# raulmur/ORB_SLAM

Hardware: NVIDIA H100
Metric: Mkeypoints/s extract+match (higher is better)
Workload: dtype u8

## Files before the change

orb_slam_b200/csrc/extract_kernels.cu:

```cuda
#include <cuda_fp16.h>

#include "orbfe_internal.h"

namespace orbfe {

__global__ void cell_select_harris_kernel(const PlanDev *__restrict__ plan, WorkDev wk, int f0);
__global__ void level_select_harris_kernel(const PlanDev *__restrict__ plan, WorkDev wk, int f0);

__device__ __forceinline__ int find_level_by(const PlanDev *plan, int idx, int which) {
    int l = 0;
    const int n = plan->nlevels;
    for (int k = 1; k < n; k++) {
        const LevelDev &L = plan->lv[k];
        const int base = which == 0 ? L.ftile_base : which == 1 ? L.btile_base : which == 2 ? L.cell_base : L.kp_base;
        if (idx >= base) l = k;
    }
    return l;
}

__device__ __forceinline__ void pdl_prologue() {
    asm volatile("griddepcontrol.launch_dependents;" ::: "memory");
    asm volatile("griddepcontrol.wait;" ::: "memory");
}

// ... 107 lines not shown
#undef RZ_PIX_SEL
#undef RZ_MIX
        if (y < dh) *reinterpret_cast<uint32_t *>(dst + (size_t)y * D.pitch) = out;
    }
}

void launch_resize_level(const PlanDev *d_plan, const PlanDev &hp, int level, int f0, int nf, cudaStream_t s) {
    const LevelDev &D = hp.lv[level];
    dim3 block(64, 4);
    dim3 grid((D.w + 255) / 256, (D.h + 4 * RZ_ROWS - 1) / (4 * RZ_ROWS), nf);
    launch_k(resize_level_kernel, grid, block, 0, s, hp.pdl != 0, d_plan, level, f0);
}

#define F2_W ORBFE_FT_W
#define F2_H ORBFE_FT_H
#define F2_PW 144
#define F2_PWORDS 35
#define F2_PH (F2_H + 8)
#define F2_MS 128
#ifndef ORBFE_FAST_ARC_DEFAULT
#define ORBFE_FAST_ARC_DEFAULT 12
#endif
#define F2_MH (F2_H + 2)
static_assert(F2_MH == 64, "the m tile is 8 warps x 8 rows; row 64 does not exist (ti.hmask has 64 bits)");

__device__ __forceinline__ uint32_t max16_u16x2(const uint32_t *w) {
    const uint32_t a0 = __vimax3_u16x2(w[0], w[1], w[2]), a1 = __vimax3_u16x2(w[3], w[4], w[5]);
    const uint32_t a2 = __vimax3_u16x2(w[6], w[7], w[8]), a3 = __vimax3_u16x2(w[9], w[10], w[11]);
    const uint32_t a4 = __vimax3_u16x2(w[12], w[13], w[14]);
    return __vmaxu2(__vimax3_u16x2(a0, a1, a2), __vimax3_u16x2(a3, a4, w[15]));
}
__device__ __forceinline__ uint32_t min16_u16x2(const uint32_t *w) {
    const uint32_t a0 = __vimin3_u16x2(w[0], w[1], w[2]), a1 = __vimin3_u16x2(w[3], w[4], w[5]);
    const uint32_t a2 = __vimin3_u16x2(w[6], w[7], w[8]), a3 = __vimin3_u16x2(w[9], w[10], w[11]);
    const uint32_t a4 = __vimin3_u16x2(w[12], w[13], w[14]);
    return __vminu2(__vimin3_u16x2(a0, a1, a2), __vimin3_u16x2(a3, a4, w[15]));
}

__device__ __forceinline__ uint32_t fast_m_u16x2(const uint32_t (&r)[16], uint32_t c) {
    uint32_t tmin[16], tmax[16], w[16];
#pragma unroll
    for (int k = 0; k < 16; k++) {
        tmin[k] = __vimin3_u16x2(r[k], r[(k + 1) & 15], r[(k + 2) & 15]);
        tmax[k] = __vimax3_u16x2(r[k], r[(k + 1) & 15], r[(k + 2) & 15]);
    }
#pragma unroll
    for (int k = 0; k < 16; k++) w[k] = __vimin3_u16x2(tmin[k], tmin[(k + 3) & 15], tmin[(k + 6) & 15]);
// ... 62 lines not shown
template <int ARC>
__device__ __forceinline__ uint32_t fast_m_arc(const uint32_t (&r)[16], uint32_t c) {
    if (ARC < 0) return fast_m_u16x2(r, c);
    return fast_m2_u16x2<(ARC < 0 ? 0 : ARC)>(r, c);
}

__device__ __forceinline__ void fast_load_row(const uint8_t *row , uint32_t (&P)[8]) {
    const uint32_t w0 = *reinterpret_cast<const uint32_t *>(row);
    const uint32_t w1 = *reinterpret_cast<const uint32_t *>(row + 4);
    const uint32_t w2 = *reinterpret_cast<const uint32_t *>(row + 8);
    const uint32_t E0 = __byte_perm(w0, 0, 0x4240), O0 = __byte_perm(w0, 0, 0x4341);
    const uint32_t E1 = __byte_perm(w1, 0, 0x4240), O1 = __byte_perm(w1, 0, 0x4341);
    const uint32_t E2 = __byte_perm(w2, 0, 0x4240), O2 = __byte_perm(w2, 0, 0x4341);
    P[0] = O0;
    P[1] = __byte_perm(E0, E1, 0x5412);
    P[2] = __byte_perm(O0, O1, 0x5412);
    P[3] = E1;
    P[4] = O1;
    P[5] = __byte_perm(E1, E2, 0x5412);
    P[6] = __byte_perm(O1, O2, 0x5412);
    P[7] = E2;
}

__device__ __forceinline__ int m_at(const uint32_t *mt, int r, int c ) {
    const int g = c >> 2, k = c & 3;
    const uint32_t wv = mt[(r * 32 + g) * 2 + (k & 1)];
    return (k & 2) ? (int)(wv >> 16) : (int)(wv & 0xFFFF);
}

#define F2_MAXC ((F2_W / 2) * (F2_H / 2) + 4 * (F2_W + F2_H))
#define F2_MAXCELLS 64

__device__ __forceinline__ uint32_t float_order_key(float v) {
    const uint32_t b = __float_as_uint(v);
    return (b & 0x80000000u) ? ~b : (b | 0x80000000u);
}
__device__ __forceinline__ float float_from_order_key(uint32_t k) {
    return __uint_as_float((k & 0x80000000u) ? (k & 0x7FFFFFFFu) : ~k);
}

__device__ __forceinline__ float harris_response(const uint8_t *__restrict__ img, int pitch, int x, int y, float scale4) {
    int a = 0, b = 0, c = 0;
    for (int i = -3; i <= 3; i++) {
        const uint8_t *r0 = img + (size_t)(y + i - 1) * pitch + x, *r1 = r0 + pitch, *r2 = r1 + pitch;
        for (int j = -3; j <= 3; j++) {
            const int Ix = ((int)__ldg(r1 + j + 1) - (int)__ldg(r1 + j - 1)) * 2 + ((int)__ldg(r0 + j + 1) - (int)__ldg(r0 + j - 1)) +
                           ((int)__ldg(r2 + j + 1) - (int)__ldg(r2 + j - 1));
            const int Iy = ((int)__ldg(r2 + j) - (int)__ldg(r0 + j)) * 2 + ((int)__ldg(r2 + j - 1) - (int)__ldg(r0 + j - 1)) +
                           ((int)__ldg(r2 + j + 1) - (int)__ldg(r0 + j + 1));
            a += Ix * Ix;
            b += Iy * Iy;
// ... 2 lines not shown
    }
    const float fa = (float)a, fb = (float)b, fc = (float)c;
    const float s = __fadd_rn(fa, fb);
    const float t = __fsub_rn(__fsub_rn(__fmul_rn(fa, fb), __fmul_rn(fc, fc)), __fmul_rn(__fmul_rn(0.04f, s), s));
    return __fmul_rn(t, scale4);
}

__device__ __forceinline__ void fast_push(uint32_t *q, int *q_n, int xl, int yl, int m) {
    const int n = atomicAdd(q_n, 1);
    q[n] = (uint32_t)xl | ((uint32_t)yl << 7) | ((uint32_t)m << 13);
}

__device__ __forceinline__ void cell_window(const LevelDev &L, int xmax, int ymax, int x, int y, int &ci, int &cj, int &xa,
                                            int &xb, int &ya, int &yb) {
    cj = min((int)__umulhi((uint32_t)(x - ORBFE_EDGE), L.cw_rcp), L.cols - 1);
    ci = min((int)__umulhi((uint32_t)(y - ORBFE_EDGE), L.ch_rcp), L.rows - 1);
    xa = ORBFE_EDGE + cj * L.cw;
    ya = ORBFE_EDGE + ci * L.ch;
    xb = (cj == L.cols - 1) ? xmax - 1 : xa + L.cw - 1;
    yb = (ci == L.rows - 1) ? ymax - 1 : ya + L.ch - 1;
}

template <int PSTRIDE, int ARC>
__device__ __forceinline__ void fast_tile_compute(const PlanDev *__restrict__ plan, const WorkDev &wk, int tile, int level, int f, int x0, int y0, const uint8_t *pix, uint32_t *mt,
                                                  uint32_t *s_cand, int &s_n, int *s_cnt_lo, int *s_cnt_hi,
                                                  long long *s_kbase, int *s_klim) {
    const int tlo = plan->t_lo;
    const int g = threadIdx.x & 31, seg = threadIdx.x >> 5;
    const int gx = x0 - 4 + 4 * g;
    {
        const int xmax = plan->lv[level].w - ORBFE_EDGE, ymax = plan->lv[level].h - ORBFE_EDGE;
        uint32_t keepA = 0, keepB = 0;
        if (gx >= ORBFE_EDGE && gx < xmax) keepA |= 0x00003C00u;
        if (gx + 2 >= ORBFE_EDGE && gx + 2 < xmax) keepA |= 0x3C000000u;
        if (gx + 1 >= ORBFE_EDGE && gx + 1 < xmax) keepB |= 0x00003C00u;
        if (gx + 3 >= ORBFE_EDGE && gx + 3 < xmax) keepB |= 0x3C000000u;
        const uint32_t ntlo2 = (uint32_t)tlo * 0x00010001u | 0x80008000u;
        uint32_t yin_bits = 0;
#pragma unroll
        for (int i = 0; i < 8; i++) {
            const int y = y0 - 1 + seg * 8 + i;
            if (y >= ORBFE_EDGE && y < ymax) yin_bits |= 1u << i;
        }
        const uint8_t *base = &pix[(seg * 8) * PSTRIDE + 4 * g];
        uint32_t P[7][8];
#pragma unroll
        for (int r = 0; r < 6; r++) fast_load_row(base + r * PSTRIDE, P[r]);
#pragma unroll
        for (int i = 0; i < 8; i++) {
            fast_load_row(base + (6 + i) * PSTRIDE, P[(6 + i) % 7]);
#define FROW(dy) P[(i + (dy) + 3) % 7]
            uint32_t mA, mB;
            {
                const uint32_t r[16] = {FROW(3)[3], FROW(3)[4], FROW(2)[5], FROW(1)[6], FROW(0)[6], FROW(-1)[6], FROW(-2)[5], FROW(-3)[4],
                                        FROW(-3)[3], FROW(-3)[2], FROW(-2)[1], FROW(-1)[0], FROW(0)[0], FROW(1)[0], FROW(2)[1], FROW(3)[2]};
                mA = fast_m_arc<ARC>(r, FROW(0)[3]);
            }
            {
                const uint32_t r[16] = {FROW(3)[4], FROW(3)[5], FROW(2)[6], FROW(1)[7], FROW(0)[7], FROW(-1)[7], FROW(-2)[6], FROW(-3)[5],
                                        FROW(-3)[4], FROW(-3)[3], FROW(-2)[2], FROW(-1)[1], FROW(0)[1], FROW(1)[1], FROW(2)[2], FROW(3)[3]};
                mB = fast_m_arc<ARC>(r, FROW(0)[4]);
            }
#undef FROW
            const int mr = seg * 8 + i;
            const bool yin = (yin_bits >> i) & 1u;
            uint2 o;
            o.x = hfma2_relu(mA, yin ? keepA : 0u, ntlo2);
            o.y = hfma2_relu(mB, yin ? keepB : 0u, ntlo2);
            *reinterpret_cast<uint2 *>(&mt[(mr * 32 + g) * 2]) = o;
        }
    }
    __syncthreads();
    const FTileInfo &ti = wk.ftile_info[tile];
    const LevelDev &L = plan->lv[ti.level];
    const int xmax = L.w - ORBFE_EDGE, ymax = L.h - ORBFE_EDGE;
    const int thi = plan->t_hi;
    uint32_t fbits = 0;
    const int r0 = seg * 8;
    uint32_t vb;
    {
        const uint32_t nib = (ti.vmask[g >> 3] >> (4 * (g & 7))) & 15u;
        vb = nib | (__shfl_down_sync(0xffffffffu, nib, 1) & 1u) << 4;
    }
    if (g >= 1 && g <= 30) {
        const uint32_t ONE2 = 0x3C003C00u, NEG2 = 0xBC00BC00u;
        const uint32_t kLA = ((vb & 1u) ? 0u : 0x00003C00u) | ((vb & 4u) ? 0u : 0x3C000000u);
        const uint32_t kM = ((vb & 2u) ? 0u : 0x00003C00u) | ((vb & 8u) ? 0u : 0x3C000000u);
        const uint32_t kRB = ((vb & 4u) ? 0u : 0x00003C00u) | ((vb & 16u) ? 0u : 0x3C000000u);
        const uint32_t nkM = kM | 0x80008000u;
        const uint32_t hm = (uint32_t)(ti.hmask >> r0);
        uint32_t A[3], B[3], lrA[3], lrB[3], fullA[3], fullB[3];
#pragma unroll
        for (int j = 0; j < 10; j++) {
            const int rr = j == 0 ? max(r0 - 1, 0) : j == 9 ? min(r0 + 8, F2_MH - 1) : r0 - 1 + j;
            const uint32_t *rowp = &mt[(rr * 32 + g) * 2];
            const uint2 own = *reinterpret_cast<const uint2 *>(rowp);
            const uint32_t pB = rowp[-1], nA = rowp[2];
            const int sl = j % 3;
            A[sl] = own.x;
            B[sl] = own.y;
            const uint32_t leftA = hmul2(__byte_perm(pB, own.y, 0x5432), kLA);
            const uint32_t rightB = hmul2(__byte_perm(own.x, nA, 0x5432), kRB);
            lrA[sl] = hmax2_keep(leftA, own.y, kM, nkM);
            fullA[sl] = hmax2_keep(lrA[sl], own.x, ONE2, NEG2);
            lrB[sl] = hmax2_keep(rightB, own.x, kM, nkM);
            fullB[sl] = hmax2_keep(lrB[sl], own.y, ONE2, NEG2);
            if (j >= 2) {
                const int c = (j - 1) % 3, u = (j - 2) % 3, d = j % 3;
                const uint32_t kUp = ((hm >> (j - 2)) & 1u) ? 0u : ONE2, kDn = ((hm >> (j - 1)) & 1u) ? 0u : ONE2;
                const uint32_t eA = hfma2(A[c], NEG2, hmax2_keep(hmax2_keep(lrA[c], fullA[d], kDn, kDn | 0x80008000u), fullA[u], kUp, kUp | 0x80008000u));
                const uint32_t eB = hfma2(B[c], NEG2, hmax2_keep(hmax2_keep(lrB[c], fullB[d], kDn, kDn | 0x80008000u), fullB[u], kUp, kUp | 0x80008000u));
                fbits |= (__byte_perm(eA, eB, 0x7351) & 0x80808080u) >> (7 - (j - 2));
            }
        }
        if (seg == 0) fbits &= 0xFEFEFEFEu;
        if (seg == 7) fbits &= 0x7F7F7F7Fu;
    }
    {
        {
            const int mine = __popc(fbits);
            int incl = mine;
#pragma unroll
            for (int o = 1; o < 32; o <<= 1) {
                const int v = __shfl_up_sync(0xffffffffu, incl, o);
                if (g >= o) incl += v;
            }
            int wbase = 0;
            const int total = __shfl_sync(0xffffffffu, incl, 31);
            if (g == 31 && total) wbase = atomicAdd(&s_n, total);
            wbase = __shfl_sync(0xffffffffu, wbase, 31);
            int n = wbase + incl - mine;
            while (fbits) {
                const int b = __ffs(fbits) - 1;
                fbits &= fbits - 1;
                const int cr = r0 + (b & 7), k = b >> 3;
                s_cand[n++] = (uint32_t)(gx + k - x0) | ((uint32_t)(cr - 1) << 7) | ((uint32_t)(m_at(mt, cr, 4 * g + k) + tlo) << 13);
            }
        }
    }
    __syncthreads();
    const int ncand = s_n;
    const int ncell_loc = ti.ncj * ti.nci;
    for (int i = threadIdx.x; i < ncand; i += blockDim.x) {
        const uint32_t q = s_cand[i];
        const int x = x0 + (int)(q & 127), y = y0 + (int)((q >> 7) & 63), m = (int)((q >> 13) & 255);
        int ci, cj, xa, xb, ya, yb;
        cell_window(L, xmax, ymax, x, y, ci, cj, xa, xb, ya, yb);
        const int lc = (ci - ti.ci0) * ti.ncj + (cj - ti.cj0);
        const int slot = atomicAdd(&s_cnt_lo[lc], 1);
        if (m > thi) atomicAdd(&s_cnt_hi[lc], 1);
        if (slot >= 2048) atomicExch(wk.err_flag, 3);
        s_cand[i] = q | ((uint32_t)slot << 21);
    }
    __syncthreads();
    if ((int)threadIdx.x < ncell_loc) {
        const int lc = threadIdx.x;
        const int gcell = L.cell_base + (ti.ci0 + lc / ti.ncj) * L.cols + (ti.cj0 + lc % ti.ncj);
        const size_t fc = (size_t)f * plan->ncells_total + gcell;
        const int cap = wk.cell_cand_cap[gcell];
// ... 7 lines not shown
        s_klim[lc] = cap - base;
    }
    __syncthreads();
    for (int i = threadIdx.x; i < ncand; i += blockDim.x) {
        const uint32_t q = s_cand[i];
        const int x = x0 + (int)(q & 127), y = y0 + (int)((q >> 7) & 63), m = (int)((q >> 13) & 255), slot = (int)(q >> 21);
        int ci, cj, xa, xb, ya, yb;
        cell_window(L, xmax, ymax, x, y, ci, cj, xa, xb, ya, yb);
        const int lc = (ci - ti.ci0) * ti.ncj + (cj - ti.cj0);
        const uint32_t raster = (uint32_t)((y - ya) * L.cw + (x - xa));
        if (slot < s_klim[lc]) {
            const size_t kidx = (size_t)(s_kbase[lc] + slot);
            if (wk.cand_keys64) {
                const float resp = harris_response(L.pyr + (size_t)f * L.plane, L.pitch, x, y, plan->harris_scale4);
                wk.cand_keys64[kidx] = ((unsigned long long)float_order_key(resp) << 32) |
                                       ((unsigned long long)(0xFFFFFFu - raster) << 8) | (unsigned long long)(m - 1);
            } else {
                wk.cand_keys[kidx] = ((uint32_t)(m - 1) << 24) | (0xFFFFFFu - raster);
            }
        }
    }
}

__global__ void __launch_bounds__(256, 2) fast_nms_kernel(const PlanDev *__restrict__ plan, WorkDev wk, int f0) {
    __shared__ __align__(16) uint8_t sbuf[(F2_MAXC * 4 > F2_PH * F2_PW) ? F2_MAXC * 4 : F2_PH * F2_PW];
    __shared__ __align__(16) uint32_t mt[F2_MH * 32 * 2];
    __shared__ int s_n, s_cnt_lo[F2_MAXCELLS], s_cnt_hi[F2_MAXCELLS], s_klim[F2_MAXCELLS];
    __shared__ long long s_kbase[F2_MAXCELLS];
    uint8_t *pix = sbuf;
    uint32_t *s_cand = reinterpret_cast<uint32_t *>(sbuf);

    const int f = blockIdx.y + f0;
    const FTileInfo ti = wk.ftile_info[blockIdx.x];
    const LevelDev &L = plan->lv[ti.level];
    const int x0 = ORBFE_EDGE + ti.tx * F2_W, y0 = ORBFE_EDGE + ti.ty * F2_H;
    const int h = L.h, pitch = L.pitch;
    const uint8_t *__restrict__ img = L.pyr + (size_t)f * L.plane;

    if (threadIdx.x < F2_MAXCELLS) { s_cnt_lo[threadIdx.x] = 0; s_cnt_hi[threadIdx.x] = 0; }
    if (threadIdx.x == 0) s_n = 0;
    {
        const int max_word = pitch / 4 - 1;
        const int wx0 = (x0 - 8) >> 2;
        for (int i = threadIdx.x; i < F2_PH * F2_PWORDS; i += blockDim.x) {
            const int r = i / F2_PWORDS, c = i - r * F2_PWORDS;
            const int gy = min(y0 - 4 + r, h - 1);
            const int gw = min(wx0 + c, max_word);
            *reinterpret_cast<uint32_t *>(&pix[r * F2_PW + c * 4]) =
                __ldg(reinterpret_cast<const uint32_t *>(img + (size_t)gy * pitch) + gw);
        }
    }
    __syncthreads();
    fast_tile_compute<F2_PW, ORBFE_FAST_ARC_DEFAULT>(plan, wk, blockIdx.x, ti.level, f, x0, y0, pix, mt, s_cand, s_n, s_cnt_lo, s_cnt_hi, s_kbase, s_klim);
}

__device__ __forceinline__ uint32_t smem_u32(const void *p) { return (uint32_t)__cvta_generic_to_shared(p); }

__device__ __forceinline__ void mbar_init(uint64_t *bar, int count) {
    asm volatile("mbarrier.init.shared::cta.b64 [%0], %1;" ::"r"(smem_u32(bar)), "r"(count));
}
__device__ __forceinline__ void mbar_expect_tx(uint64_t *bar, uint32_t bytes) {
    asm volatile("mbarrier.arrive.expect_tx.shared::cta.b64 _, [%0], %1;" ::"r"(smem_u32(bar)), "r"(bytes) : "memory");
}
__device__ __forceinline__ void mbar_wait(uint64_t *bar, uint32_t parity) {
    asm volatile(
        "{\n"
        ".reg .pred p;\n"
        "WAIT_%=:\n"
        "mbarrier.try_wait.parity.shared::cta.b64 p, [%0], %1;\n"
        "@p bra DONE_%=;\n"
        "bra WAIT_%=;\n"
        "DONE_%=:\n"
        "}\n" ::"r"(smem_u32(bar)), "r"(parity) : "memory");
}
__device__ __forceinline__ void tma_load_3d(void *smem_dst, const void *tmap, uint64_t *bar, int c0, int c1, int c2) {
    asm volatile(
        "cp.async.bulk.tensor.3d.shared::cluster.global.mbarrier::complete_tx::bytes [%0], [%1, {%3, %4, %5}], [%2];"
        ::"r"(smem_u32(smem_dst)), "l"(tmap), "r"(smem_u32(bar)), "r"(c0), "r"(c1), "r"(c2) : "memory");
}

#define F2_TW 160
#define F2_PIXBYTES (F2_PH * F2_TW)
#define F2_PIXSLOT ((F2_PIXBYTES + 127) / 128 * 128)
#define F2_TMA_SMEM (2 * F2_PIXSLOT + F2_MH * 32 * 2 * 4 + 128)
static_assert(F2_MAXC * 4 <= F2_PIXSLOT, "the candidate queue lives in the pixel slot that was just consumed");

template <int ARC, int MINB>
__global__ void __launch_bounds__(256, MINB) fast_nms_tma_kernel(const PlanDev *__restrict__ plan, WorkDev wk, int f0, int nwork) {
    extern __shared__ __align__(128) uint8_t dsm[];
    uint8_t *pixbuf0 = dsm, *pixbuf1 = dsm + F2_PIXSLOT;
    uint32_t *mt = reinterpret_cast<uint32_t *>(dsm + 2 * F2_PIXSLOT);
    __shared__ __align__(8) uint64_t bar[2];
    __shared__ int s_n, s_cnt_lo[F2_MAXCELLS], s_cnt_hi[F2_MAXCELLS], s_klim[F2_MAXCELLS];
    __shared__ long long s_kbase[F2_MAXCELLS];

    const int ntiles = plan->nftiles_total;
    if (threadIdx.x == 0) {
        mbar_init(&bar[0], 1);
        mbar_init(&bar[1], 1);
        asm volatile("fence.mbarrier_init.release.cluster;" ::: "memory");
    }
    __syncthreads();
    pdl_prologue();
    int wi = blockIdx.x;
    if (wi < nwork && threadIdx.x == 0) {
        const FTileInfo t0 = wk.ftile_info[wi % ntiles];
        mbar_expect_tx(&bar[0], F2_PIXBYTES);
        tma_load_3d(pixbuf0, &wk.tmaps[t0.level], &bar[0], (ORBFE_EDGE + t0.tx * F2_W - 8) & ~15, ORBFE_EDGE + t0.ty * F2_H - 4, f0 + wi / ntiles);
    }
    for (int it = 0; wi < nwork; it++, wi += gridDim.x) {
        const int cur = it & 1;
        const int nxt = wi + gridDim.x;
        const FTileInfo ti = wk.ftile_info[wi % ntiles];
        const int f = f0 + wi / ntiles;
        const int x0 = ORBFE_EDGE + ti.tx * F2_W, y0 = ORBFE_EDGE + ti.ty * F2_H;
        if (threadIdx.x < F2_MAXCELLS) { s_cnt_lo[threadIdx.x] = 0; s_cnt_hi[threadIdx.x] = 0; }
        if (threadIdx.x == 0) s_n = 0;
        mbar_wait(&bar[cur], (it >> 1) & 1);
        __syncthreads();
        if (nxt < nwork && threadIdx.x == 0) {
            const FTileInfo tn = wk.ftile_info[nxt % ntiles];
            mbar_expect_tx(&bar[cur ^ 1], F2_PIXBYTES);
            tma_load_3d(cur ? pixbuf0 : pixbuf1, &wk.tmaps[tn.level], &bar[cur ^ 1], (ORBFE_EDGE + tn.tx * F2_W - 8) & ~15,
                        ORBFE_EDGE + tn.ty * F2_H - 4, f0 + nxt / ntiles);
        }
        uint8_t *slot_cur = cur ? pixbuf1 : pixbuf0;
        fast_tile_compute<F2_TW, ARC>(plan, wk, wi % ntiles, ti.level, f, x0, y0, slot_cur + ((x0 - 8) & 15), mt, reinterpret_cast<uint32_t *>(slot_cur),
                                 s_n, s_cnt_lo, s_cnt_hi, s_kbase, s_klim);
    }
}

#define FAST_ARC_VARIANTS(X) X(-1, 4) X(0, 4) X(4, 4) X(8, 4) X(12, 4) X(16, 4) X(12, 3) X(16, 3)
typedef void (*FastTmaKernel)(const PlanDev *, WorkDev, int, int);
static FastTmaKernel fast_tma_variant(int arc, int minb) {
#define X(a, b) if (arc == (a) && minb == (b)) return fast_nms_tma_kernel<(a), (b)>;
    FAST_ARC_VARIANTS(X)
#undef X
    return nullptr;
}
int fast_arc_supported(int arc, int ctas_per_sm) { return fast_tma_variant(arc, ctas_per_sm <= 3 ? 3 : 4) != nullptr; }

int fast_tma_setup() {
#define X(a, b) { cudaError_t e = cudaFuncSetAttribute(fast_nms_tma_kernel<(a), (b)>, cudaFuncAttributeMaxDynamicSharedMemorySize, F2_TMA_SMEM); if (e != cudaSuccess) return (int)e; }
    FAST_ARC_VARIANTS(X)
#undef X
    return 0;
}

void launch_fast_nms(const PlanDev *d_plan, const PlanDev &hp, WorkDev w, int f0, int nf, cudaStream_t s) {
    if (hp.nftiles_total == 0) return;
    if (w.tmaps) {
        const int nwork = hp.nftiles_total * nf;
        const int grid = min(nwork, w.fast_grid);
        launch_k(fast_tma_variant(w.fast_arc, w.fast_ctas <= 3 ? 3 : 4), dim3(grid), dim3(256), F2_TMA_SMEM, s, hp.pdl != 0, d_plan, w, f0, nwork);
        return;
    }
    dim3 grid(hp.nftiles_total, nf);
    fast_nms_kernel<<<grid, 256, 0, s>>>(d_plan, w, f0);
}

__device__ __forceinline__ int warp_sum(int v) {
#pragma unroll
    for (int o = 16; o > 0; o >>= 1) v += __shfl_xor_sync(0xffffffffu, v, o);
    return v;
}

__global__ void __launch_bounds__(32) cell_quota_kernel(const PlanDev *__restrict__ plan, WorkDev wk, int f0) {
    pdl_prologue();
    __shared__ uint32_t no_more[128];
    const int l = blockIdx.x, f = blockIdx.y + f0;
    const LevelDev &L = plan->lv[l];
    const int lane = threadIdx.x;
    const int nCells = L.ncells, nfc = L.nfc;
    const size_t fb = (size_t)f * plan->ncells_total + L.cell_base;
    const int t1_is_lo = plan->t1_is_lo;
    const int t1 = t1_is_lo ? plan->t_lo : plan->t_hi;
    const int t2 = t1_is_lo ? plan->t_hi : plan->t_lo;
    for (int i = lane; i < 128; i += 32) no_more[i] = 0;
    __syncwarp();

    int toDist = 0, nNoMore = 0;
// ... 810 lines not shown
```

orb_slam_b200/csrc/orbfe_api.cu:

```cuda
#include <cuda.h>
#include <cuda_runtime.h>

#include <algorithm>
#include <cmath>
#include <cstdarg>
#include <cstdio>
#include <cstdlib>
#include <cstring>
#include <string>
#include <vector>
#include <atomic>
#include <thread>
#include <unordered_map>

#include "orbfe_internal.h"

using namespace orbfe;

static thread_local char g_err[512] = "";

static int fail(int code, const char *fmt, ...) {
    va_list ap;
    va_start(ap, fmt);
    vsnprintf(g_err, sizeof(g_err), fmt, ap);
// ... 297 lines not shown
        for (int l = 0; l < ex->nlevels; l++) {
            const LevelDev &L = P.lv[l];
            for (int ty = 0; ty < L.btiles_y; ty++)
                for (int tx = 0; tx < L.btiles_x; tx++) {
                    BTileInfo &T = binfo[(size_t)L.btile_base + ty * L.btiles_x + tx];
                    T.level = (short)l; T.tx = (short)tx; T.ty = (short)ty; T.pad = 0;
                }
        }
        BTileInfo *d_binfo;
        CU_TRY(dmalloc(ex, &d_binfo, binfo.size()));
        CU_TRY(cudaMemcpy(d_binfo, binfo.data(), sizeof(BTileInfo) * binfo.size(), cudaMemcpyHostToDevice));
        Wk.btile_info = d_binfo;
    }
    long long *d_cb; int *d_cc;
    CU_TRY(dmalloc(ex, &d_cb, cand_base.size()));
    CU_TRY(dmalloc(ex, &d_cc, cand_cap.size()));
    CU_TRY(cudaMemcpy(d_cb, cand_base.data(), sizeof(long long) * cand_base.size(), cudaMemcpyHostToDevice));
    CU_TRY(cudaMemcpy(d_cc, cand_cap.data(), sizeof(int) * cand_cap.size(), cudaMemcpyHostToDevice));
    Wk.cell_cand_base = d_cb;
    Wk.cell_cand_cap = d_cc;
    Wk.tmaps = nullptr;
    Wk.fast_grid = 0;
    Wk.fast_arc = ORBFE_FAST_ARC_RUNTIME_DEFAULT;
    Wk.fast_ctas = getenv("ORBFE_FAST_CTAS") ? std::max(1, atoi(getenv("ORBFE_FAST_CTAS"))) : 3;
    if (const char *a = getenv("ORBFE_FAST_ARC")) Wk.fast_arc = atoi(a);
    if (!fast_arc_supported(Wk.fast_arc, Wk.fast_ctas))
        return fail(ORBFE_ERR_ARG, "ORBFE_FAST_ARC=%d with ORBFE_FAST_CTAS=%d is not a compiled variant of the FAST kernel", Wk.fast_arc, Wk.fast_ctas);
    if (!getenv("ORBFE_FAST_NO_TMA")) {
        typedef CUresult (*EncodeFn)(CUtensorMap *, CUtensorMapDataType, cuuint32_t, void *, const cuuint64_t *, const cuuint64_t *,
                                     const cuuint32_t *, const cuuint32_t *, CUtensorMapInterleave, CUtensorMapSwizzle,
                                     CUtensorMapL2promotion, CUtensorMapFloatOOBfill);
        void *fn = nullptr;
        cudaDriverEntryPointQueryResult qres;
        if (cudaGetDriverEntryPoint("cuTensorMapEncodeTiled", &fn, cudaEnableDefault, &qres) != cudaSuccess || !fn ||
            qres != cudaDriverEntryPointSuccess)
            return fail(ORBFE_ERR_CUDA, "cuTensorMapEncodeTiled is not available from this driver");
        std::vector<CUtensorMap> maps(ex->nlevels);
        for (int l = 0; l < ex->nlevels; l++) {
            const LevelDev &L = P.lv[l];
            const cuuint64_t dims[3] = {(cuuint64_t)L.w, (cuuint64_t)L.h, (cuuint64_t)B};
            const cuuint64_t strides[2] = {(cuuint64_t)L.pitch, (cuuint64_t)L.plane};
            const cuuint32_t box[3] = {160, ORBFE_FT_H + 8, 1};
            const cuuint32_t estr[3] = {1, 1, 1};
            CUresult r = ((EncodeFn)fn)(&maps[l], CU_TENSOR_MAP_DATA_TYPE_UINT8, 3, L.pyr, dims, strides, box, estr,
                                        CU_TENSOR_MAP_INTERLEAVE_NONE, CU_TENSOR_MAP_SWIZZLE_NONE, CU_TENSOR_MAP_L2_PROMOTION_L2_128B,
                                        CU_TENSOR_MAP_FLOAT_OOB_FILL_NONE);
            if (r != CUDA_SUCCESS) return fail(ORBFE_ERR_CUDA, "cuTensorMapEncodeTiled(level %d) failed: %d", l, (int)r);
        }
        CUtensorMap *d_maps;
        CU_TRY(dmalloc(ex, &d_maps, maps.size()));
        CU_TRY(cudaMemcpy(d_maps, maps.data(), sizeof(CUtensorMap) * maps.size(), cudaMemcpyHostToDevice));
        Wk.tmaps = d_maps;
        ex->tma_encode = fn;
        ex->d_maps = d_maps;
        cudaError_t e = (cudaError_t)fast_tma_setup();
        if (e != cudaSuccess) return fail(ORBFE_ERR_CUDA, "cudaFuncSetAttribute(fast_nms_tma_kernel): %s", cudaGetErrorString(e));
        int nsm = 132;
        cudaDeviceGetAttribute(&nsm, cudaDevAttrMultiProcessorCount, ex->device);
        Wk.fast_grid = Wk.fast_ctas * nsm;
    }
    CU_TRY(dmalloc(ex, &Wk.cand_keys, (size_t)cand_total * B));
    if (ex->score_type == 0) {
        CU_TRY(dmalloc(ex, &Wk.cand_keys64, (size_t)cand_total * B));
        CU_TRY(dmalloc(ex, &Wk.kept_aux, (size_t)P.kept_total * B));
    }
    const size_t nc = (size_t)P.ncells_total * B, nl = (size_t)P.nlevels * B;
    int *cnt;
    ex->counters_bytes = sizeof(int) * (2 * nc + nl);
    CU_TRY(dmalloc(ex, &cnt, 2 * nc + nl));
    ex->counters = cnt;
    Wk.cell_cnt_lo = cnt;
    Wk.cell_cnt_hi = cnt + nc;
    Wk.kept_cnt = cnt + 2 * nc;
    CU_TRY(dmalloc(ex, &Wk.cell_keep, nc));
    CU_TRY(dmalloc(ex, &Wk.cell_min_key, nc));
    CU_TRY(dmalloc(ex, &Wk.kept_keys, (size_t)P.kept_total * B));
    CU_TRY(dmalloc(ex, &Wk.kp_xy_score, (size_t)std::max(P.nfeatures, 1) * B));
    CU_TRY(dmalloc(ex, &Wk.level_cnt, nl));
    CU_TRY(dmalloc(ex, &Wk.err_flag, 1));
    CU_TRY(cudaMemsetAsync(Wk.err_flag, 0, sizeof(int), ex->stream));
    CU_TRY(dmalloc(ex, &ex->d_kps, (size_t)std::max(P.nfeatures, 1) * B));
    CU_TRY(dmalloc(ex, &ex->d_desc, (size_t)std::max(P.nfeatures, 1) * B * 32));
// ... 1042 lines not shown
```

orb_slam_b200/csrc/orbfe_internal.h:

```cpp
#pragma once

#include <cuda.h>
#include <cuda_runtime.h>
#include <stdint.h>

#include "../../include/orbfe.h"

#define ORBFE_EDGE 16

#define ORBFE_FT_W 120
#define ORBFE_FT_H 62
#define ORBFE_FAST_ARC_RUNTIME_DEFAULT 16
#define ORBFE_BT_W 120
#define ORBFE_BT_H 64

namespace orbfe {

struct LevelDev {
    uint8_t *pyr;
    uint8_t *blur;
    size_t plane;
    int w, h, pitch;
    int cols, rows, cw, ch, ncells, nfc, quota;
    uint32_t cw_rcp, ch_rcp;
    int cell_base;
    int kp_base;
    int kept_base, kept_cap;
    int ftiles_x, ftiles_y, ftile_base;
    int btiles_x, btiles_y, btile_base;
    float scale;
    float patch_size;
    const int *xofs;
    const short2 *xab;
    const int2 *yrows;
    const short2 *yab;
// ... 7 lines not shown
    int t1_is_lo;
    int score_type;
    int pdl;
    float harris_scale4;
    long long cand_total;
    LevelDev lv[ORBFE_MAX_LEVELS];
};

struct FTileInfo {
    short cj0, ci0, ncj, nci;
    short level, tx, ty, pad;
    unsigned long long hmask;
    unsigned int vmask[4];
};
struct BTileInfo { short level, tx, ty, pad; };

struct WorkDev {
    const long long *cell_cand_base;
    const int *cell_cand_cap;
    const FTileInfo *ftile_info;
    const BTileInfo *btile_info;
    const CUtensorMap *tmaps;
    int fast_grid;
    int fast_ctas;
    int fast_arc;
    uint32_t *cand_keys;
    unsigned long long *cand_keys64;
    uint32_t *kept_aux;
    int *cell_cnt_lo;
    int *cell_cnt_hi;
    int *cell_keep;
    uint32_t *cell_min_key;
    unsigned long long *kept_keys;
    int *kept_cnt;
    int2 *kp_xy_score;
    int *level_cnt;
    int *err_flag;
};

#define ORBFE_MAX_PEERS 16
struct PeerOut {
    int n;
    unsigned epoch;
    unsigned *done;
    const unsigned *ack;
    unsigned ack_epoch;
    int *err;
    OrbfeKeyPoint *kps[ORBFE_MAX_PEERS];
    uint8_t *desc[ORBFE_MAX_PEERS];
    int *counts[ORBFE_MAX_PEERS];
    unsigned *flag[ORBFE_MAX_PEERS];
};

void launch_resize_level(const PlanDev *d_plan, const PlanDev &h_plan, int level, int f0, int nf, cudaStream_t s);
void launch_fast_nms(const PlanDev *d_plan, const PlanDev &h_plan, WorkDev w, int f0, int nf, cudaStream_t s);
void launch_cell_quota(const PlanDev *d_plan, const PlanDev &h_plan, WorkDev w, int f0, int nf, cudaStream_t s);
void launch_cell_select(const PlanDev *d_plan, const PlanDev &h_plan, WorkDev w, int f0, int nf, cudaStream_t s);
void launch_level_select(const PlanDev *d_plan, const PlanDev &h_plan, WorkDev w, size_t smem_bytes, int f0, int nf, cudaStream_t s);
void launch_blur(const PlanDev *d_plan, const PlanDev &h_plan, WorkDev w, int f0, int nf, int dst_f0, cudaStream_t s);
void launch_describe(const PlanDev *d_plan, const PlanDev &h_plan, WorkDev w, const int8_t *d_pattern,
                     OrbfeKeyPoint *d_kps, uint8_t *d_desc, int *d_counts, int f0, int nf, cudaStream_t s);
void launch_describe_fused(const PlanDev *d_plan, const PlanDev &h_plan, WorkDev w, const int8_t *d_pattern,
                     OrbfeKeyPoint *d_kps, uint8_t *d_desc, int *d_counts, int f0, int nf, cudaStream_t s, const PeerOut *peers = nullptr);
int fast_tma_setup();
int fast_arc_supported(int arc, int ctas_per_sm);
int level_select_smem_bytes(int max_kept);
int level_select_harris_smem_bytes(int max_kept);
int set_level_select_harris_smem(int bytes);
int set_level_select_smem(int bytes);

struct SbpParams {
    float min_x, min_y, max_x, max_y, gw, gh;
    float fx, fy, cx, cy, th;
    float scale[ORBFE_MAX_LEVELS];
    int nlevels, cap, check_ori;
    int qcap;
    int rule, th_dist;
    float nnratio;
    int scratch_per_pair;
    int smem_entries;
    int smem_fixed;
    const unsigned *xw_flags;
    unsigned *xw_ack[16];
    unsigned *xw_done;
    int *xw_err;
    int xw_n;
    unsigned xw_epoch;
};
// ... 25 lines not shown
```

Baseline: 46.71.

## Fuse FAST NMS into score loop with 4 warps of 16 rows

The FAST tile kernel now uses 128 threads, each warp covering 16 rows, and runs the 3x3 non-max suppression in registers while scores are computed. This removes the separate shared-memory pass over the score tile. Only u8 scores are stored to shared memory, for the warp-boundary rows and the candidate score lookup. Launch bounds now come from a register budget, and the grid size is taken from the occupancy API. The trade-offs are higher register pressure, fewer threads per tile, and extra boundary-row fixups after a sync.

```diff
diff --git a/orb_slam_b200/csrc/extract_kernels.cu b/orb_slam_b200/csrc/extract_kernels.cu
--- a/orb_slam_b200/csrc/extract_kernels.cu
+++ b/orb_slam_b200/csrc/extract_kernels.cu
@@ -153,7 +153,8 @@
 #define ORBFE_FAST_ARC_DEFAULT 12
 #endif
 #define F2_MH (F2_H + 2)
-static_assert(F2_MH == 64, "the m tile is 8 warps x 8 rows; row 64 does not exist (ti.hmask has 64 bits)");
+#define F2_THREADS 128
+static_assert(F2_MH == 4 * 16, "the m tile is 4 warps x 16 rows; row 64 does not exist (ti.hmask has 64 bits)");
 
 __device__ __forceinline__ uint32_t max16_u16x2(const uint32_t *w) {
     const uint32_t a0 = __vimax3_u16x2(w[0], w[1], w[2]), a1 = __vimax3_u16x2(w[3], w[4], w[5]);
@@ -262,11 +263,23 @@
     P[7] = E2;
 }
 
-__device__ __forceinline__ int m_at(const uint32_t *mt, int r, int c ) {
-    const int g = c >> 2, k = c & 3;
-    const uint32_t wv = mt[(r * 32 + g) * 2 + (k & 1)];
-    return (k & 2) ? (int)(wv >> 16) : (int)(wv & 0xFFFF);
-}
+__device__ __forceinline__ int s_at(const uint32_t *st, int r, int c ) {
+    return reinterpret_cast<const uint8_t *>(st)[r * F2_MS + c];
+}
+
+__device__ __forceinline__ void nms_row(uint32_t A, uint32_t B, uint32_t kLA, uint32_t kM, uint32_t kRB, uint32_t &lrA,
+                                        uint32_t &lrB, uint32_t &fullA, uint32_t &fullB) {
+    const uint32_t ONE2 = 0x3C003C00u, NEG2 = 0xBC00BC00u, nkM = kM | 0x80008000u;
+    const uint32_t pB = __shfl_up_sync(0xffffffffu, B, 1);
+    const uint32_t nA = __shfl_down_sync(0xffffffffu, A, 1);
+    const uint32_t leftA = hmul2(__byte_perm(pB, B, 0x5432), kLA);
+    const uint32_t rightB = hmul2(__byte_perm(A, nA, 0x5432), kRB);
+    lrA = hmax2_keep(leftA, B, kM, nkM);
+    fullA = hmax2_keep(lrA, A, ONE2, NEG2);
+    lrB = hmax2_keep(rightB, A, kM, nkM);
+    fullB = hmax2_keep(lrB, B, ONE2, NEG2);
+}
+__device__ __forceinline__ uint32_t nms_beats(uint32_t eA, uint32_t eB) { return __byte_perm(eA, eB, 0x7351) & 0x80808080u; }
 
 #define F2_MAXC ((F2_W / 2) * (F2_H / 2) + 4 * (F2_W + F2_H))
 #define F2_MAXCELLS 64
@@ -315,12 +328,24 @@
 }
 
 template <int PSTRIDE, int ARC>
-__device__ __forceinline__ void fast_tile_compute(const PlanDev *__restrict__ plan, const WorkDev &wk, int tile, int level, int f, int x0, int y0, const uint8_t *pix, uint32_t *mt,
+__device__ __forceinline__ void fast_tile_compute(const PlanDev *__restrict__ plan, const WorkDev &wk, int tile, int level, int f, int x0, int y0, const uint8_t *pix, uint32_t *st,
                                                   uint32_t *s_cand, int &s_n, int *s_cnt_lo, int *s_cnt_hi,
                                                   long long *s_kbase, int *s_klim) {
     const int tlo = plan->t_lo;
     const int g = threadIdx.x & 31, seg = threadIdx.x >> 5;
     const int gx = x0 - 4 + 4 * g;
+    const int r0 = seg * 16;
+    const FTileInfo &ti = wk.ftile_info[tile];
+    const uint32_t ONE2 = 0x3C003C00u, NEG2 = 0xBC00BC00u;
+    uint32_t kLA, kM, kRB;
+    {
+        const uint32_t nib = (ti.vmask[g >> 3] >> (4 * (g & 7))) & 15u;
+        const uint32_t vb = nib | (__shfl_down_sync(0xffffffffu, nib, 1) & 1u) << 4;
+        kLA = ((vb & 1u) ? 0u : 0x00003C00u) | ((vb & 4u) ? 0u : 0x3C000000u);
+        kM = ((vb & 2u) ? 0u : 0x00003C00u) | ((vb & 8u) ? 0u : 0x3C000000u);
+        kRB = ((vb & 4u) ? 0u : 0x00003C00u) | ((vb & 16u) ? 0u : 0x3C000000u);
+    }
+    uint64_t fbits;
     {
         const int xmax = plan->lv[level].w - ORBFE_EDGE, ymax = plan->lv[level].h - ORBFE_EDGE;
         uint32_t keepA = 0, keepB = 0;
@@ -329,89 +354,96 @@
         if (gx + 1 >= ORBFE_EDGE && gx + 1 < xmax) keepB |= 0x00003C00u;
         if (gx + 3 >= ORBFE_EDGE && gx + 3 < xmax) keepB |= 0x3C000000u;
         const uint32_t ntlo2 = (uint32_t)tlo * 0x00010001u | 0x80008000u;
-        uint32_t yin_bits = 0;
-#pragma unroll
-        for (int i = 0; i < 8; i++) {
-            const int y = y0 - 1 + seg * 8 + i;
-            if (y >= ORBFE_EDGE && y < ymax) yin_bits |= 1u << i;
-        }
-        const uint8_t *base = &pix[(seg * 8) * PSTRIDE + 4 * g];
+        uint32_t row_bits = (uint32_t)(ti.hmask >> r0) << 16;
+#pragma unroll
+        for (int i = 0; i < 16; i++) {
+            const int y = y0 - 1 + r0 + i;
+            if (y >= ORBFE_EDGE && y < ymax) row_bits |= 1u << i;
+        }
+        const uint8_t *rowp = &pix[r0 * PSTRIDE + 4 * g];
+        uint32_t *stp = &st[r0 * 32 + g];
         uint32_t P[7][8];
-#pragma unroll
-        for (int r = 0; r < 6; r++) fast_load_row(base + r * PSTRIDE, P[r]);
-#pragma unroll
-        for (int i = 0; i < 8; i++) {
-            fast_load_row(base + (6 + i) * PSTRIDE, P[(6 + i) % 7]);
-#define FROW(dy) P[(i + (dy) + 3) % 7]
-            uint32_t mA, mB;
-            {
-                const uint32_t r[16] = {FROW(3)[3], FROW(3)[4], FROW(2)[5], FROW(1)[6], FROW(0)[6], FROW(-1)[6], FROW(-2)[5], FROW(-3)[4],
-                                        FROW(-3)[3], FROW(-3)[2], FROW(-2)[1], FROW(-1)[0], FROW(0)[0], FROW(1)[0], FROW(2)[1], FROW(3)[2]};
-                mA = fast_m_arc<ARC>(r, FROW(0)[3]);
-            }
-            {
-                const uint32_t r[16] = {FROW(3)[4], FROW(3)[5], FROW(2)[6], FROW(1)[7], FROW(0)[7], FROW(-1)[7], FROW(-2)[6], FROW(-3)[5],
-                                        FROW(-3)[4], FROW(-3)[3], FROW(-2)[2], FROW(-1)[1], FROW(0)[1], FROW(1)[1], FROW(2)[2], FROW(3)[3]};
-                mB = fast_m_arc<ARC>(r, FROW(0)[4]);
-            }
+        uint32_t cA = 0, cB = 0, accA = 0, accB = 0, fA = 0, fB = 0;
+#pragma unroll
+        for (int r = 0; r < 6; r++) fast_load_row(rowp + r * PSTRIDE, P[r]);
+        uint32_t w0 = 0, w1 = 0, w2 = 0;
+#pragma unroll 1
+        for (int b = 0; b < 3; b++) {
+            uint32_t w = 0;
+#pragma unroll
+            for (int j = 0; j < 7; j++) {
+                if (j >= 2 && b == 2) break;
+                fast_load_row(rowp + (6 + j) * PSTRIDE, P[(6 + j) % 7]);
+#define FROW(dy) P[(j + (dy) + 3) % 7]
+                uint32_t mA, mB;
+                {
+                    const uint32_t r[16] = {FROW(3)[3], FROW(3)[4], FROW(2)[5], FROW(1)[6], FROW(0)[6], FROW(-1)[6], FROW(-2)[5], FROW(-3)[4],
+                                            FROW(-3)[3], FROW(-3)[2], FROW(-2)[1], FROW(-1)[0], FROW(0)[0], FROW(1)[0], FROW(2)[1], FROW(3)[2]};
+                    mA = fast_m_arc<ARC>(r, FROW(0)[3]);
+                }
+                {
+                    const uint32_t r[16] = {FROW(3)[4], FROW(3)[5], FROW(2)[6], FROW(1)[7], FROW(0)[7], FROW(-1)[7], FROW(-2)[6], FROW(-3)[5],
+                                            FROW(-3)[4], FROW(-3)[3], FROW(-2)[2], FROW(-1)[1], FROW(0)[1], FROW(1)[1], FROW(2)[2], FROW(3)[3]};
+                    mB = fast_m_arc<ARC>(r, FROW(0)[4]);
+                }
 #undef FROW
-            const int mr = seg * 8 + i;
-            const bool yin = (yin_bits >> i) & 1u;
-            uint2 o;
-            o.x = hfma2_relu(mA, yin ? keepA : 0u, ntlo2);
-            o.y = hfma2_relu(mB, yin ? keepB : 0u, ntlo2);
-            *reinterpret_cast<uint2 *>(&mt[(mr * 32 + g) * 2]) = o;
-        }
-    }
-    __syncthreads();
-    const FTileInfo &ti = wk.ftile_info[tile];
+                const bool yin = (row_bits >> j) & 1u;
+                const uint32_t A = hfma2_relu(mA, yin ? keepA : 0u, ntlo2);
+                const uint32_t B = hfma2_relu(mB, yin ? keepB : 0u, ntlo2);
+                stp[j * 32] = __byte_perm(A, B, 0x6240);
+                uint32_t lrA, lrB, nfA, nfB;
+                nms_row(A, B, kLA, kM, kRB, lrA, lrB, nfA, nfB);
+                const uint32_t kV = ((row_bits >> (16 + j)) & 1u) ? 0u : ONE2, nkV = kV | 0x80008000u;
+                const uint32_t eA = hfma2(cA, NEG2, hmax2_keep(accA, nfA, kV, nkV));
+                const uint32_t eB = hfma2(cB, NEG2, hmax2_keep(accB, nfB, kV, nkV));
+                w |= nms_beats(eA, eB) >> (7 - j);
+                accA = hmax2_keep(lrA, fA, kV, nkV);
+                accB = hmax2_keep(lrB, fB, kV, nkV);
+                cA = A;
+                cB = B;
+                fA = nfA;
+                fB = nfB;
+            }
+            w0 = w1;
+            w1 = w2;
+            w2 = w;
+            rowp += 7 * PSTRIDE;
+            stp += 7 * 32;
+            row_bits >>= 7;
+        }
+        w2 |= nms_beats(hfma2(cA, NEG2, accA), hfma2(cB, NEG2, accB)) >> 5;
+        const uint32_t lo = (w0 >> 1) | ((w1 << 6) & 0xC0C0C0C0u);
+        const uint32_t hi = ((w1 >> 2) & 0x1F1F1F1Fu) | ((w2 << 5) & 0xE0E0E0E0u);
+        fbits = (uint64_t)hi << 32 | lo;
+    }
+    __syncthreads();
+    if (seg > 0) {
+        const uint32_t kV = ((ti.hmask >> r0) & 1u) ? 0u : ONE2;
+        const uint32_t wn = st[(r0 - 1) * 32 + g], wc = st[r0 * 32 + g];
+        uint32_t lrA, lrB, nfA, nfB;
+        nms_row(__byte_perm(wn, 0, 0x4240), __byte_perm(wn, 0, 0x4341), kLA, kM, kRB, lrA, lrB, nfA, nfB);
+        const uint32_t beats = nms_beats(hfma2(__byte_perm(wc, 0, 0x4240), NEG2, hmul2(nfA, kV)),
+                                         hfma2(__byte_perm(wc, 0, 0x4341), NEG2, hmul2(nfB, kV)));
+        fbits &= ~(uint64_t)((~beats & 0x80808080u) >> 7);
+    }
+    if (seg < 3) {
+        const uint32_t kV = ((ti.hmask >> (r0 + 16)) & 1u) ? 0u : ONE2;
+        const uint32_t wn = st[(r0 + 16) * 32 + g], wc = st[(r0 + 15) * 32 + g];
+        uint32_t lrA, lrB, nfA, nfB;
+        nms_row(__byte_perm(wn, 0, 0x4240), __byte_perm(wn, 0, 0x4341), kLA, kM, kRB, lrA, lrB, nfA, nfB);
+        const uint32_t beats = nms_beats(hfma2(__byte_perm(wc, 0, 0x4240), NEG2, hmul2(nfA, kV)),
+                                         hfma2(__byte_perm(wc, 0, 0x4341), NEG2, hmul2(nfB, kV)));
+        fbits &= ~((uint64_t)(~beats & 0x80808080u) << 32);
+    }
+    if (seg == 0) fbits &= ~0x01010101ull;
+    if (seg == 3) fbits &= ~0x8080808000000000ull;
+    if (g == 0 || g == 31) fbits = 0;
     const LevelDev &L = plan->lv[ti.level];
     const int xmax = L.w - ORBFE_EDGE, ymax = L.h - ORBFE_EDGE;
     const int thi = plan->t_hi;
-    uint32_t fbits = 0;
-    const int r0 = seg * 8;
-    uint32_t vb;
-    {
-        const uint32_t nib = (ti.vmask[g >> 3] >> (4 * (g & 7))) & 15u;
-        vb = nib | (__shfl_down_sync(0xffffffffu, nib, 1) & 1u) << 4;
-    }
-    if (g >= 1 && g <= 30) {
-        const uint32_t ONE2 = 0x3C003C00u, NEG2 = 0xBC00BC00u;
-        const uint32_t kLA = ((vb & 1u) ? 0u : 0x00003C00u) | ((vb & 4u) ? 0u : 0x3C000000u);
-        const uint32_t kM = ((vb & 2u) ? 0u : 0x00003C00u) | ((vb & 8u) ? 0u : 0x3C000000u);
-        const uint32_t kRB = ((vb & 4u) ? 0u : 0x00003C00u) | ((vb & 16u) ? 0u : 0x3C000000u);
-        const uint32_t nkM = kM | 0x80008000u;
-        const uint32_t hm = (uint32_t)(ti.hmask >> r0);
-        uint32_t A[3], B[3], lrA[3], lrB[3], fullA[3], fullB[3];
-#pragma unroll
-        for (int j = 0; j < 10; j++) {
-            const int rr = j == 0 ? max(r0 - 1, 0) : j == 9 ? min(r0 + 8, F2_MH - 1) : r0 - 1 + j;
-            const uint32_t *rowp = &mt[(rr * 32 + g) * 2];
-            const uint2 own = *reinterpret_cast<const uint2 *>(rowp);
-            const uint32_t pB = rowp[-1], nA = rowp[2];
-            const int sl = j % 3;
-            A[sl] = own.x;
-            B[sl] = own.y;
-            const uint32_t leftA = hmul2(__byte_perm(pB, own.y, 0x5432), kLA);
-            const uint32_t rightB = hmul2(__byte_perm(own.x, nA, 0x5432), kRB);
-            lrA[sl] = hmax2_keep(leftA, own.y, kM, nkM);
-            fullA[sl] = hmax2_keep(lrA[sl], own.x, ONE2, NEG2);
-            lrB[sl] = hmax2_keep(rightB, own.x, kM, nkM);
-            fullB[sl] = hmax2_keep(lrB[sl], own.y, ONE2, NEG2);
-            if (j >= 2) {
-                const int c = (j - 1) % 3, u = (j - 2) % 3, d = j % 3;
-                const uint32_t kUp = ((hm >> (j - 2)) & 1u) ? 0u : ONE2, kDn = ((hm >> (j - 1)) & 1u) ? 0u : ONE2;
-                const uint32_t eA = hfma2(A[c], NEG2, hmax2_keep(hmax2_keep(lrA[c], fullA[d], kDn, kDn | 0x80008000u), fullA[u], kUp, kUp | 0x80008000u));
-                const uint32_t eB = hfma2(B[c], NEG2, hmax2_keep(hmax2_keep(lrB[c], fullB[d], kDn, kDn | 0x80008000u), fullB[u], kUp, kUp | 0x80008000u));
-                fbits |= (__byte_perm(eA, eB, 0x7351) & 0x80808080u) >> (7 - (j - 2));
-            }
-        }
-        if (seg == 0) fbits &= 0xFEFEFEFEu;
-        if (seg == 7) fbits &= 0x7F7F7F7Fu;
-    }
     {
         {
-            const int mine = __popc(fbits);
+            const int mine = __popcll(fbits);
             int incl = mine;
 #pragma unroll
             for (int o = 1; o < 32; o <<= 1) {
@@ -424,10 +456,10 @@
             wbase = __shfl_sync(0xffffffffu, wbase, 31);
             int n = wbase + incl - mine;
             while (fbits) {
-                const int b = __ffs(fbits) - 1;
+                const int b = __ffsll(fbits) - 1;
                 fbits &= fbits - 1;
-                const int cr = r0 + (b & 7), k = b >> 3;
-                s_cand[n++] = (uint32_t)(gx + k - x0) | ((uint32_t)(cr - 1) << 7) | ((uint32_t)(m_at(mt, cr, 4 * g + k) + tlo) << 13);
+                const int cr = r0 + ((b >> 5) << 3 | (b & 7)), k = (b >> 3) & 3;
+                s_cand[n++] = (uint32_t)(gx + k - x0) | ((uint32_t)(cr - 1) << 7) | ((uint32_t)(s_at(st, cr, 4 * g + k) + tlo) << 13);
             }
         }
     }
@@ -481,9 +513,9 @@
     }
 }
 
-__global__ void __launch_bounds__(256, 2) fast_nms_kernel(const PlanDev *__restrict__ plan, WorkDev wk, int f0) {
+__global__ void __launch_bounds__(F2_THREADS, 4) fast_nms_kernel(const PlanDev *__restrict__ plan, WorkDev wk, int f0) {
     __shared__ __align__(16) uint8_t sbuf[(F2_MAXC * 4 > F2_PH * F2_PW) ? F2_MAXC * 4 : F2_PH * F2_PW];
-    __shared__ __align__(16) uint32_t mt[F2_MH * 32 * 2];
+    __shared__ __align__(16) uint32_t st[F2_MH * F2_MS / 4];
     __shared__ int s_n, s_cnt_lo[F2_MAXCELLS], s_cnt_hi[F2_MAXCELLS], s_klim[F2_MAXCELLS];
     __shared__ long long s_kbase[F2_MAXCELLS];
     uint8_t *pix = sbuf;
@@ -510,7 +542,7 @@
         }
     }
     __syncthreads();
-    fast_tile_compute<F2_PW, ORBFE_FAST_ARC_DEFAULT>(plan, wk, blockIdx.x, ti.level, f, x0, y0, pix, mt, s_cand, s_n, s_cnt_lo, s_cnt_hi, s_kbase, s_klim);
+    fast_tile_compute<F2_PW, ORBFE_FAST_ARC_DEFAULT>(plan, wk, blockIdx.x, ti.level, f, x0, y0, pix, st, s_cand, s_n, s_cnt_lo, s_cnt_hi, s_kbase, s_klim);
 }
 
 __device__ __forceinline__ uint32_t smem_u32(const void *p) { return (uint32_t)__cvta_generic_to_shared(p); }
@@ -541,14 +573,14 @@
 #define F2_TW 160
 #define F2_PIXBYTES (F2_PH * F2_TW)
 #define F2_PIXSLOT ((F2_PIXBYTES + 127) / 128 * 128)
-#define F2_TMA_SMEM (2 * F2_PIXSLOT + F2_MH * 32 * 2 * 4 + 128)
+#define F2_TMA_SMEM (2 * F2_PIXSLOT + F2_MH * F2_MS + 128)
 static_assert(F2_MAXC * 4 <= F2_PIXSLOT, "the candidate queue lives in the pixel slot that was just consumed");
 
-template <int ARC, int MINB>
-__global__ void __launch_bounds__(256, MINB) fast_nms_tma_kernel(const PlanDev *__restrict__ plan, WorkDev wk, int f0, int nwork) {
+template <int ARC, int REGS>
+__global__ void __launch_bounds__(F2_THREADS, 65536 / (F2_THREADS * REGS)) fast_nms_tma_kernel(const PlanDev *__restrict__ plan, WorkDev wk, int f0, int nwork) {
     extern __shared__ __align__(128) uint8_t dsm[];
     uint8_t *pixbuf0 = dsm, *pixbuf1 = dsm + F2_PIXSLOT;
-    uint32_t *mt = reinterpret_cast<uint32_t *>(dsm + 2 * F2_PIXSLOT);
+    uint32_t *st = reinterpret_cast<uint32_t *>(dsm + 2 * F2_PIXSLOT);
     __shared__ __align__(8) uint64_t bar[2];
     __shared__ int s_n, s_cnt_lo[F2_MAXCELLS], s_cnt_hi[F2_MAXCELLS], s_klim[F2_MAXCELLS];
     __shared__ long long s_kbase[F2_MAXCELLS];
@@ -584,20 +616,24 @@
                         ORBFE_EDGE + tn.ty * F2_H - 4, f0 + nxt / ntiles);
         }
         uint8_t *slot_cur = cur ? pixbuf1 : pixbuf0;
-        fast_tile_compute<F2_TW, ARC>(plan, wk, wi % ntiles, ti.level, f, x0, y0, slot_cur + ((x0 - 8) & 15), mt, reinterpret_cast<uint32_t *>(slot_cur),
+        fast_tile_compute<F2_TW, ARC>(plan, wk, wi % ntiles, ti.level, f, x0, y0, slot_cur + ((x0 - 8) & 15), st, reinterpret_cast<uint32_t *>(slot_cur),
                                  s_n, s_cnt_lo, s_cnt_hi, s_kbase, s_klim);
     }
 }
 
-#define FAST_ARC_VARIANTS(X) X(-1, 4) X(0, 4) X(4, 4) X(8, 4) X(12, 4) X(16, 4) X(12, 3) X(16, 3)
+#define FAST_ARC_VARIANTS(X) X(-1, 64) X(0, 64) X(4, 64) X(8, 64) X(12, 64) X(16, 64) X(12, 80) X(16, 80) X(12, 96) X(16, 96)
 typedef void (*FastTmaKernel)(const PlanDev *, WorkDev, int, int);
-static FastTmaKernel fast_tma_variant(int arc, int minb) {
-#define X(a, b) if (arc == (a) && minb == (b)) return fast_nms_tma_kernel<(a), (b)>;
+static FastTmaKernel fast_tma_variant(int arc, int regs) {
+#define X(a, b) if (arc == (a) && regs == (b)) return fast_nms_tma_kernel<(a), (b)>;
     FAST_ARC_VARIANTS(X)
 #undef X
     return nullptr;
 }
-int fast_arc_supported(int arc, int ctas_per_sm) { return fast_tma_variant(arc, ctas_per_sm <= 3 ? 3 : 4) != nullptr; }
+int fast_arc_supported(int arc, int regs) { return fast_tma_variant(arc, regs) != nullptr; }
+
+int fast_tma_ctas_per_sm(int arc, int regs, int *ctas) {
+    return (int)cudaOccupancyMaxActiveBlocksPerMultiprocessor(ctas, fast_tma_variant(arc, regs), F2_THREADS, F2_TMA_SMEM);
+}
 
 int fast_tma_setup() {
 #define X(a, b) { cudaError_t e = cudaFuncSetAttribute(fast_nms_tma_kernel<(a), (b)>, cudaFuncAttributeMaxDynamicSharedMemorySize, F2_TMA_SMEM); if (e != cudaSuccess) return (int)e; }
@@ -611,11 +647,11 @@
     if (w.tmaps) {
         const int nwork = hp.nftiles_total * nf;
         const int grid = min(nwork, w.fast_grid);
-        launch_k(fast_tma_variant(w.fast_arc, w.fast_ctas <= 3 ? 3 : 4), dim3(grid), dim3(256), F2_TMA_SMEM, s, hp.pdl != 0, d_plan, w, f0, nwork);
+        launch_k(fast_tma_variant(w.fast_arc, w.fast_regs), dim3(grid), dim3(F2_THREADS), F2_TMA_SMEM, s, hp.pdl != 0, d_plan, w, f0, nwork);
         return;
     }
     dim3 grid(hp.nftiles_total, nf);
-    fast_nms_kernel<<<grid, 256, 0, s>>>(d_plan, w, f0);
+    fast_nms_kernel<<<grid, F2_THREADS, 0, s>>>(d_plan, w, f0);
 }
 
 __device__ __forceinline__ int warp_sum(int v) {
diff --git a/orb_slam_b200/csrc/orbfe_api.cu b/orb_slam_b200/csrc/orbfe_api.cu
--- a/orb_slam_b200/csrc/orbfe_api.cu
+++ b/orb_slam_b200/csrc/orbfe_api.cu
@@ -343,10 +343,11 @@
     Wk.tmaps = nullptr;
     Wk.fast_grid = 0;
     Wk.fast_arc = ORBFE_FAST_ARC_RUNTIME_DEFAULT;
-    Wk.fast_ctas = getenv("ORBFE_FAST_CTAS") ? std::max(1, atoi(getenv("ORBFE_FAST_CTAS"))) : 3;
+    Wk.fast_regs = ORBFE_FAST_REGS_DEFAULT;
+    if (const char *c = getenv("ORBFE_FAST_CTAS")) Wk.fast_regs = std::max(1, atoi(c)) <= 3 ? 80 : 64;
     if (const char *a = getenv("ORBFE_FAST_ARC")) Wk.fast_arc = atoi(a);
-    if (!fast_arc_supported(Wk.fast_arc, Wk.fast_ctas))
-        return fail(ORBFE_ERR_ARG, "ORBFE_FAST_ARC=%d with ORBFE_FAST_CTAS=%d is not a compiled variant of the FAST kernel", Wk.fast_arc, Wk.fast_ctas);
+    if (!fast_arc_supported(Wk.fast_arc, Wk.fast_regs))
+        return fail(ORBFE_ERR_ARG, "ORBFE_FAST_ARC=%d with %d registers is not a compiled variant of the FAST kernel", Wk.fast_arc, Wk.fast_regs);
     if (!getenv("ORBFE_FAST_NO_TMA")) {
         typedef CUresult (*EncodeFn)(CUtensorMap *, CUtensorMapDataType, cuuint32_t, void *, const cuuint64_t *, const cuuint64_t *,
                                      const cuuint32_t *, const cuuint32_t *, CUtensorMapInterleave, CUtensorMapSwizzle,
@@ -378,7 +379,10 @@
         if (e != cudaSuccess) return fail(ORBFE_ERR_CUDA, "cudaFuncSetAttribute(fast_nms_tma_kernel): %s", cudaGetErrorString(e));
         int nsm = 132;
         cudaDeviceGetAttribute(&nsm, cudaDevAttrMultiProcessorCount, ex->device);
-        Wk.fast_grid = Wk.fast_ctas * nsm;
+        int per_sm = 0;
+        e = (cudaError_t)fast_tma_ctas_per_sm(Wk.fast_arc, Wk.fast_regs, &per_sm);
+        if (e != cudaSuccess || per_sm < 1) return fail(ORBFE_ERR_CUDA, "fast_nms_tma_kernel does not fit on an SM: %s", cudaGetErrorString(e));
+        Wk.fast_grid = per_sm * nsm;
     }
     CU_TRY(dmalloc(ex, &Wk.cand_keys, (size_t)cand_total * B));
     if (ex->score_type == 0) {
diff --git a/orb_slam_b200/csrc/orbfe_internal.h b/orb_slam_b200/csrc/orbfe_internal.h
--- a/orb_slam_b200/csrc/orbfe_internal.h
+++ b/orb_slam_b200/csrc/orbfe_internal.h
@@ -11,6 +11,7 @@
 #define ORBFE_FT_W 120
 #define ORBFE_FT_H 62
 #define ORBFE_FAST_ARC_RUNTIME_DEFAULT 16
+#define ORBFE_FAST_REGS_DEFAULT 96
 #define ORBFE_BT_W 120
 #define ORBFE_BT_H 64
 
@@ -64,7 +65,7 @@
     const BTileInfo *btile_info;
     const CUtensorMap *tmaps;
     int fast_grid;
-    int fast_ctas;
+    int fast_regs;
     int fast_arc;
     uint32_t *cand_keys;
     unsigned long long *cand_keys64;
@@ -105,7 +106,8 @@
 void launch_describe_fused(const PlanDev *d_plan, const PlanDev &h_plan, WorkDev w, const int8_t *d_pattern,
                      OrbfeKeyPoint *d_kps, uint8_t *d_desc, int *d_counts, int f0, int nf, cudaStream_t s, const PeerOut *peers = nullptr);
 int fast_tma_setup();
-int fast_arc_supported(int arc, int ctas_per_sm);
+int fast_arc_supported(int arc, int regs);
+int fast_tma_ctas_per_sm(int arc, int regs, int *ctas);
 int level_select_smem_bytes(int max_kept);
 int level_select_harris_smem_bytes(int max_kept);
 int set_level_select_harris_smem(int bytes);
```

Result: faster. 48.04, median of 6 (+2.8%).
